# om-ai-lab/OmChat

Measured on AMD Instinct MI355X. Metric: images/sec prefill + decode tokens/sec, OmChat-13B TP=1/8; p50 TTFT, higher is better.
Workload: dtype bf16

## Files before the change

omchat_amd/csrc/capi.hip:

```cpp
#include "kernels.h"
#include <stdlib.h>
#include "../../include/omchat_hip.h"
#include <math.h>
#include <vector>

#define S(x) ((hipStream_t)(x))
#if OMCHAT_EXPERIMENTS
int g_launch_any_order = 0;
#endif

extern "C" int omchat_op_gemm(int dtype, const void* A, int lda, const void* W, int ldw, void* C, int ldc, int M, int N, int K,
                              const void* bias, const void* ls, const void* resid, int ldr, int epi, int force_tile, void* stream) {
  GemmArgs g{A, lda, W, ldw, C, ldc, M, N, K, bias, ls, resid, ldr, epi, force_tile, nullptr, 0, -1};
  return launch_gemm(dtype, g, S(stream));
}

extern "C" int omchat_op_gemm_fused(int dtype, const void* A, int lda, const void* W, int ldw, void* C, int ldc, int M, int N, int K,
                                    const void* bias, const void* ls, const void* resid, int ldr, int epi, int force_tile, const float* row_scale,
                                    const float* rs_stats, int rs_ld, int rs_nslots, int rs_dim, float rs_eps,
                                    float* stats, int stats_ld, int* nslots, void* stream) {
  GemmArgs g{A, lda, W, ldw, C, ldc, M, N, K, bias, ls, resid, ldr, epi, force_tile, nullptr, 0, -1};
  g.row_scale = row_scale; g.stats = stats; g.stats_ld = stats_ld; g.stats_nslots = nslots;
  g.rs_stats = rs_stats; g.rs_ld = rs_ld; g.rs_nslots = rs_nslots; g.rs_dim = rs_dim; g.rs_eps = rs_eps;
  return launch_gemm(dtype, g, S(stream));
}
extern "C" int omchat_op_stats_finish(const float* stats, int ld, int slot0, int nslots, int ngroups, int rows, int dim, float eps, float* out, void* stream) {
  return launch_stats_finish(stats, ld, slot0, nslots, ngroups, rows, dim, eps, out, S(stream));
}
extern "C" int omchat_op_row_sumsq(int dtype, const void* x, int ldx, int rows, int H, float* stats, void* stream) {
  return launch_row_sumsq(dtype, x, ldx, rows, H, stats, S(stream));
}
extern "C" int omchat_op_fold_cols(int dtype, const void* W, const void* n, void* out, int rows, int cols, void* stream) {
  return launch_fold_cols(dtype, W, n, out, rows, cols, S(stream));
}
extern "C" int omchat_op_vit_knorm_slots(int dtype, void* k, int ld, const void* wk, int rows, int C, int C_total, float eps, const float* stats, int stats_ld,
                                         int nslots, float* sumsq_q, void* stream) {
  return launch_vit_knorm_slots(dtype, k, ld, wk, rows, C, C_total, eps, stats, stats_ld, nslots, sumsq_q, S(stream));
}
extern "C" int omchat_op_mha_qnorm(int dtype, const void* qkv, int B, int Sq, int H, const float* sumsq, int stride, int dim, const void* wq,
                                   float eps, float q_scale, void* out, void* stream) {
  OM_CHECK(qkv && out && sumsq && wq, "null argument");
  AttnArgs a{};
  const int64_t row = (int64_t)3 * H * 128;
  a.Q = qkv; a.q_sb = Sq * row; a.q_sh = 128; a.q_sr = row;
  a.K = (const char*)qkv + (size_t)H * 128 * 2; a.k_sb = a.q_sb; a.k_sh = 128; a.k_sr = row;
  a.V = (const char*)qkv + (size_t)2 * H * 128 * 2; a.v_sb = a.q_sb; a.v_sh = 128; a.v_sr = row;
  a.O = out; a.o_sb = (int64_t)Sq * H * 128; a.o_sh = 128; a.o_sr = (int64_t)H * 128;
  a.batch = B; a.q_heads = H; a.kv_heads = H; a.Sq = Sq; a.Skv = Sq; a.kv_len = nullptr; a.causal = 0; a.q_pos0 = 0;
  a.scale = 1.0f;
  a.qn_sumsq = sumsq; a.qn_stride = stride; a.qn_dim = dim; a.qn_w = wq; a.qn_eps = eps; a.qn_scale = q_scale;
  return launch_attn_prefill(dtype, a, S(stream));
}

extern "C" int omchat_op_set_tuning(int key, int value) {
  const char* allow = getenv("OMCHAT_ALLOW_TUNING");
  if (!allow || allow[0] != '1') {
    omchat_set_error("omchat_op_set_tuning: process-global test / measurement hook; set OMCHAT_ALLOW_TUNING=1 to use it (see include/omchat_hip.h)");
    return 1;
  }
  if (key == 0) { gemm_set_skew(value); return 0; }
  if (key == 1) { gemv_set_force_mfma(value); return 0; }
  if (key == 5) { gemm_set_autotune(value); return 0; }
  if (key == 4) { model_set_ar_min_rows(value); return 0; }
  if (key == 6) { model_set_pack_replica(value); return 0; }
  if (key == 8) { attn_set_v2(value); return 0; }
  if (key == 9) { model_set_fuse_peer_norm(value); return 0; }
  if (key == 10) { attn_set_tpw(value); return 0; }
  if (key == 11) { gemv_set_no_xs(value); return 0; }
  if (key == 12) { attn_set_klds(value); return 0; }
  if (key == 25) { attn_set_dma(value); return 0; }
  if (key == 26) { attn_set_dma_slots(value); return 0; }
  if (key == 27) { attn_set_dma_rot(value); return 0; }
  if (key == 28) { gemv_set_skew(value); return 0; }
  if (key == 29) { model_set_tp_f32(value); return 0; }
  if (key == 30) { attn_set_hsplit(value); return 0; }
  if (key == 33) { attn_set_mha_xcd(value); return 0; }
  if (key == 16) { gemv_set_norm_loop(value); return 0; }
  if (key == 17) { gemv_set_rows_balance(value); return 0; }
  if (key == 19) { attn_set_merge_mid_min(value); return 0; }
  if (key == 21) { attn_set_merge_dg(value); return 0; }
  if (key == 13) { gemm_set_persist(value); return 0; }
  if (key == 14) { model_set_norm_in_gemv(value); return 0; }
  if (key == 22) { model_set_fuse_attn_oproj(value); return 0; }
  if (key == 23) { model_set_decode_layer(value); return 0; }
  if (key == 24) { gemv_set_dyn(value); return 0; }
  if (key == 34) { gemv_set_shard_shapes(value); return 0; }
  if (key == 35) { model_set_shard_as_tp1(value); return 0; }
  if (key == 36) { attn_set_kg(value); return 0; }
  if (key == 37) { gemm_set_wide_store(value); return 0; }
  if (key == 43) { gemm_set_skip_dead(value); return 0; }
  if (key == 44) { model_set_vit_fused(value); return 0; }
  if (key == 45) { model_set_tp_sp(value); return 0; }
  if (key == 46) { attn_set_peel(value); return 0; }
  if (key == 47) { attn_set_kv8_tpw(value); return 0; }
  if (key == 48) { attn_set_kv8_fuse(value); return 0; }
  if (key == 49) { model_set_extend_attn(value); return 0; }
  if (key == 38) { gemv_set_gu_rr(value); return 0; }
  if (key == 39) { gemv_set_longk_direct(value); return 0; }
  if (key == 40) { norm_set_wave(value); return 0; }
#if OMCHAT_EXPERIMENTS
  if (key == 41) { g_launch_any_order = value; return 0; }
  if (key == 42) { model_set_ao_oproj(value); return 0; }
#endif
  omchat_set_error("omchat_op_set_tuning: unknown key");
  return 1;
}

extern "C" int omchat_allreduce_noop(void*, void*, size_t, int, void*) { return 0; }

extern "C" int omchat_gemm_tune_load(const char* path) { OM_CHECK(path, "null path"); return gemm_tune_load(path); }
extern "C" int omchat_gemm_tune_dump(const char* path) { OM_CHECK(path, "null path"); return gemm_tune_dump(path); }
extern "C" long omchat_gemm_tune_runs(void) { return gemm_tune_runs(); }

extern "C" size_t omchat_op_gemm_sk_ws(void) { return gemm_sk_ws_bytes(); }

extern "C" int omchat_op_gemm_sk(int dtype, const void* A, int lda, const void* W, int ldw, void* C, int ldc, int M, int N, int K,
                                 const void* bias, const void* ls, const void* resid, int ldr, int epi, int force_tile, void* ws,
                                 size_t ws_bytes, int stream_k, void* stream) {
  GemmArgs g{A, lda, W, ldw, C, ldc, M, N, K, bias, ls, resid, ldr, epi, force_tile, ws, ws_bytes, stream_k};
  return launch_gemm(dtype, g, S(stream));
}

extern "C" int omchat_op_gemv(int dtype, const void* X, int ldx, const void* W, int ldw, void* Y, int ldy, int b, int N, int K,
                              const void* bias, const void* resid, int ldr, int epi, int out_f32, void* stream) {
  GemvArgs g{X, ldx, W, ldw, Y, ldy, b, N, K, bias, resid, ldr, epi, out_f32};
  return launch_gemv(dtype, g, S(stream));
}

extern "C" int omchat_op_gemv_norm(int dtype, const void* X, const void* W, int ldw, void* Y, int N, int K, const void* norm_w, float eps,
                                   const void* bias, int epi, int out_f32, void* stream) {
  OM_CHECK(X && W && Y && norm_w, "null argument");
  GemvArgs g{X, K, W, ldw, Y, N, 1, N, K, bias, nullptr, 0, epi, out_f32};
  g.norm_w = norm_w; g.norm_eps = eps;
  return launch_gemv(dtype, g, S(stream));
}

extern "C" int omchat_op_gemv_packed(int dtype, const void* X, int ldx, const void* W, int ldw, void* Y, int ldy, int b, int N, int K,
                                     const void* bias, int epi, int out_f32, int ksplit, int w_packed, int y_packed, void* stream) {
  OM_CHECK(b >= 1 && b <= 32 && K % 64 == 0, "1 <= b <= 32, K % 64 == 0");
  const int NB = b > 16 ? 2 : 1;
  void *xp = nullptr, *wp = nullptr;
  OM_HIP(hipMalloc(&xp, (size_t)NB * 16 * K * 2));
  int rc = launch_pack_x(dtype, X, ldx, b, K, xp, S(stream));
  if (rc == 0 && w_packed) {
    if (hipMalloc(&wp, (size_t)N * K * 2) != hipSuccess) { hipFree(xp); omchat_set_error("hipMalloc failed"); return 2; }
    rc = launch_pack_w(dtype, W, ldw, N, K, wp, S(stream));
  }
  if (rc == 0) {
    GemvArgs g{xp, K, w_packed ? wp : W, ldw, Y, ldy, b, N, K, bias, nullptr, 0, epi, out_f32, ksplit, 0, nullptr, 1, w_packed, y_packed};
    rc = launch_gemv(dtype, g, S(stream));
  }
  hipStreamSynchronize(S(stream));
  hipFree(xp); if (wp) hipFree(wp);
  return rc;
}
extern "C" int omchat_op_pack_x(int dtype, const void* X, int ldx, int b, int K, void* out, void* stream) { return launch_pack_x(dtype, X, ldx, b, K, out, S(stream)); }

extern "C" int omchat_op_gemm_fp8(int dtype, const void* A8, const float* a_scale, const void* W8, const float* w_scale, void* C, int ldc, int M,
                                  int N, int K, const void* bias, const void* resid, int ldr, int epi, void* stream) {
  GemmArgs g{A8, K, W8, K, C, ldc, M, N, K, bias, nullptr, resid, ldr, epi, 0, nullptr, 0, -1, 1, a_scale, w_scale};
  return launch_gemm(dtype, g, S(stream));
}
extern "C" int omchat_op_quant_rows_fp8(int dtype, const void* x, const void* norm_w, float eps, void* y8, float* scale, int rows, int H, void* stream) {
  if (norm_w) return launch_rmsnorm_q8(dtype, x, H, norm_w, y8, H, scale, rows, H, eps, S(stream));
  return launch_quant_rows_q8(dtype, x, H, y8, H, scale, rows, H, S(stream));
}

extern "C" int omchat_op_resid_rmsnorm(int dtype, void* x, int ldx, const float* part, int ks, const void* w, void* xn, int ldn, int rows, int H,
                                       float eps, int pack_nb, void* stream) {
  OM_CHECK(x && part, "null argument");
  return launch_resid_rmsnorm(dtype, x, ldx, part, ks, w, xn, ldn, rows, H, eps, S(stream), pack_nb);
}
extern "C" int omchat_op_rmsnorm(int dtype, const void* x, const void* w, void* y, int rows, int H, float eps, void* stream) {
// ... 339 lines not shown
```

omchat_amd/csrc/gemm.hip:

```cpp
#include "kernels.h"
#include <array>
#include <stdio.h>
#include <stdlib.h>
#include <limits.h>
#include <algorithm>
#include <map>
#include <mutex>

namespace {

int g_gemm_wide_store = 1;
int g_gemm_skip_dead = 1;

struct GemmP {
  const void* A; const void* W; void* C; const void* bias; const void* ls; const void* resid;
  int lda, ldw, ldc, ldr, M, N, K;
  const float* a_scale; const float* w_scale;
  int wide_store;
  int skip_dead;
  const float* row_scale;
  float* stats; int stats_ld;
  const float* rs_stats; int rs_ld, rs_nslots; float rs_inv_dim, rs_eps;
  int rs_dma;
};

constexpr int GROUP_M = 4;
__device__ __forceinline__ int xcd_remap(int bid, int nwg) {
  const int xcd = bid & 7, q8 = nwg >> 3, r8 = nwg & 7;
  return (xcd < r8 ? xcd * (q8 + 1) : r8 * (q8 + 1) + (xcd - r8) * q8) + (bid >> 3);
}
__device__ __forceinline__ void tile_coords_id(int wgid, int M, int N, int BM, int BN, int& m0, int& n0) {
  const int tiles_m = (M + BM - 1) / BM, tiles_n = (N + BN - 1) / BN;
  const int per_group = GROUP_M * tiles_n;
  const int g = wgid / per_group, in_g = wgid % per_group;
  const int rows_here = tiles_m - g * GROUP_M < GROUP_M ? tiles_m - g * GROUP_M : GROUP_M;
  m0 = (g * GROUP_M + in_g % rows_here) * BM;
  n0 = (in_g / rows_here) * BN;
}
__device__ __forceinline__ void tile_coords(int M, int N, int BM, int BN, int& m0, int& n0) {
  tile_coords_id(xcd_remap(blockIdx.x, gridDim.x), M, N, BM, BN, m0, n0);
}

typedef const __attribute__((address_space(1))) void* gptr_t;
typedef __attribute__((address_space(3))) void* lptr_t;

template <typename T> __device__ __forceinline__ unsigned short bits16(T v) { return __builtin_bit_cast(unsigned short, v); }
template <typename T> __device__ __forceinline__ float from_bits16(unsigned short v) { return tof(__builtin_bit_cast(T, v)); }
template <typename T> __device__ __forceinline__ u32x2 pack4(float a, float b, float c, float d) {
  typename V8<T>::half_type h = {fromf<T>(a), fromf<T>(b), fromf<T>(c), fromf<T>(d)};
  return __builtin_bit_cast(u32x2, h);
}
template <typename T> __device__ __forceinline__ f32x4 unpack4(u32x2 w) {
  const typename V8<T>::half_type h = __builtin_bit_cast(typename V8<T>::half_type, w);
  return (f32x4){tof(h[0]), tof(h[1]), tof(h[2]), tof(h[3])};
}
template <typename T> __device__ __forceinline__ f32x4 load4(const T* p) {
  return unpack4<T>(*reinterpret_cast<const u32x2*>(p));
}

template <typename T, int MR, int NR, int EPI_, bool F8 = false>
__device__ __forceinline__ void gemm_epilogue(const GemmP& p, f32x4 (&acc)[MR][NR], int rowu_, int colu_, int fg, int fr, const float* rs_lds = nullptr) {
#pragma clang fp contract(off)
  constexpr bool STATS = EPI_ == EPI_LS_RESID_STATS || EPI_ == EPI_NONE_STATS;
  constexpr int EPI = EPI_ == EPI_LS_RESID_STATS ? EPI_LS_RESID : (EPI_ == EPI_NONE_STATS ? EPI_NONE : EPI_);
  const int rowu = __builtin_amdgcn_readfirstlane(rowu_), colu = __builtin_amdgcn_readfirstlane(colu_);
  const int rows_valid = p.M - rowu < MR * 16 ? p.M - rowu : MR * 16;
  if (rows_valid <= 0) return;
  if (p.row_scale || rs_lds) {
    float rs[MR];
#pragma unroll
    for (int i = 0; i < MR; ++i) {
      const int row = rowu + i * 16 + fr;
      rs[i] = rs_lds ? rs_lds[i * 16 + fr] : p.row_scale[row < p.M ? row : p.M - 1];
    }
#pragma unroll
    for (int i = 0; i < MR; ++i)
#pragma unroll
      for (int j = 0; j < NR; ++j) acc[i][j] *= rs[i];
  }
  float ssq[MR];
#pragma unroll
  for (int i = 0; i < MR; ++i) ssq[i] = 0.f;
  if constexpr (F8) {
    float sa[MR];
#pragma unroll
    for (int i = 0; i < MR; ++i) { const int row = rowu + i * 16 + fr; sa[i] = p.a_scale[row < p.M ? row : p.M - 1]; }
#pragma unroll
    for (int j = 0; j < NR; ++j) {
      const int col = colu + j * 16 + 4 * fg;
      const f32x4 sw = col < p.N ? *reinterpret_cast<const f32x4*>(p.w_scale + col) : (f32x4){0.f, 0.f, 0.f, 0.f};
#pragma unroll
      for (int i = 0; i < MR; ++i) acc[i][j] *= sw * sa[i];
    }
  }
// ... 91 lines not shown
#pragma unroll
          for (int jj = 0; jj < JG; jj += 2) {
            const int j = j0 + jj;
            if (j + 1 < NR && colu + j * 16 < p.N) {
              const bool mine = colu + (j + (fg & 1)) * 16 + 4 * (fg & ~1) < p.N;
              const int cw = (fr * p.ldc + 4 * (fg & ~1)) * 2 + (colu + (j + (fg & 1)) * 16) * 2;
              const u32x2 a = out4(i, jj), b = out4(i, jj + 1);
              const auto s0 = __builtin_amdgcn_permlane16_swap(a[0], b[0], false, false);
              const auto s1 = __builtin_amdgcn_permlane16_swap(a[1], b[1], false, false);
              const u32x4 w = {s0[0], s1[0], s0[1], s1[1]};
              if (mine) __builtin_amdgcn_raw_buffer_store_b128(w, crs, cw + i * 16 * p.ldc * 2, 0, 0);
            }
          }
        }
      } else {
#pragma unroll
      for (int jj = 0; jj < JG; ++jj) {
        const int j = j0 + jj;
        const int col = colu + j * 16 + 4 * fg;
        if (j < NR && col < p.N) {
          const int cj = c_lane + (colu + j * 16) * 2;
#pragma unroll
          for (int i = 0; i < MR; ++i) __builtin_amdgcn_raw_buffer_store_b64(out4(i, jj), crs, cj + i * 16 * p.ldc * 2, 0, 0);
        }
      }
      }
    }
    if constexpr (STATS) {
      if (colu < p.N) {
        const int slot = colu / (NR * 16);
#pragma unroll
        for (int i = 0; i < MR; ++i) {
          float v = ssq[i];
          v += __shfl_xor(v, 16);
          v += __shfl_xor(v, 32);
          const int row = rowu + i * 16 + fr;
          if (fg == 0 && row < p.M) p.stats[(size_t)slot * p.stats_ld + row] = v;
        }
      }
    }
  }
}

template <int BM, int NT>
__device__ __forceinline__ void tile_row_scale_prefetch(const GemmP& p, int m0, float* Ls) {
  const int lane = threadIdx.x & 63, wave = __builtin_amdgcn_readfirstlane((int)threadIdx.x >> 6);
  constexpr int G = (BM + 63) / 64;
  for (int pc = wave; pc < p.rs_nslots * G; pc += NT / 64) {
    const int sl = pc / G, g = pc - sl * G;
    int r = g * 64 + lane; r = r < BM ? r : BM - 1;
    int row = m0 + r; row = row < p.M ? row : p.M - 1;
    __builtin_amdgcn_global_load_lds((gptr_t)(p.rs_stats + (size_t)sl * p.rs_ld + row), (lptr_t)(Ls + sl * (G * 64) + g * 64), 4, 0, 0);
  }
}

template <int BM, int NT>
__device__ __forceinline__ void tile_row_scale(const GemmP& p, int m0, float* L, const float* Ls) {
  constexpr int TPR = NT >= 2 * BM ? 2 : 1;
  constexpr int G64 = (BM + 63) / 64 * 64;
  const int tid = threadIdx.x, h = tid / BM, r = tid % BM;
  if (h < TPR) {
    int row = m0 + r; row = row < p.M ? row : p.M - 1;
    const int per = (p.rs_nslots + TPR - 1) / TPR, s0 = h * per, s1 = s0 + per < p.rs_nslots ? s0 + per : p.rs_nslots;
    const float* base = p.rs_stats + row;
    float t = 0.f;
    for (int c0 = s0; c0 < s1; c0 += 16) {
      float v[16];
#pragma unroll
      for (int k = 0; k < 16; ++k) v[k] = c0 + k < s1 ? (Ls ? Ls[(c0 + k) * G64 + r] : base[(size_t)(c0 + k) * p.rs_ld]) : 0.f;
#pragma unroll
      for (int k = 0; k < 16; ++k) t += v[k];
    }
    L[h * BM + r] = t;
  }
  __syncthreads();
  if (tid < BM) {
    float t = L[tid];
    if (TPR == 2) t += L[BM + tid];
    L[tid] = rsqrtf(t * p.rs_inv_dim + p.rs_eps);
  }
  __syncthreads();
}

template <typename T, int BM, int BN, int WM, int WN, int EPI>
__global__ __launch_bounds__(WM* WN * 64) void gemm_kernel(GemmP p) {
  constexpr int NT = WM * WN * 64;
  constexpr int WTM = BM / WM, WTN = BN / WN;
  constexpr int MR = WTM / 16, NR = WTN / 16;
  constexpr int A_BYTES = BM * 128, B_BYTES = BN * 128, STAGE = A_BYTES + B_BYTES;
  constexpr int A_ROUNDS = (BM * 8 + NT - 1) / NT, B_ROUNDS = (BN * 8 + NT - 1) / NT;
  static_assert((BM * 8) % 64 == 0 && (BN * 8) % 64 == 0 && WTM % 16 == 0 && WTN % 16 == 0, "tile geometry");
  typedef typename V8<T>::type frag_t;
  extern __shared__ __attribute__((aligned(256))) char smem[];

  const int tid = threadIdx.x;
  const int lane = tid & 63;
  const int wave = __builtin_amdgcn_readfirstlane(tid >> 6);
  const int wm = wave / WN, wn = wave % WN;

  int m0, n0;
  tile_coords(p.M, p.N, BM, BN, m0, n0);

  const T* __restrict__ A = (const T*)p.A;
  const T* __restrict__ W = (const T*)p.W;

  const T* a_src[A_ROUNDS];
  const T* b_src[B_ROUNDS];
#pragma unroll
  for (int i = 0; i < A_ROUNDS; ++i) {
    const int lin = i * NT + tid, row = lin >> 3, pc = lin & 7;
    const int c = pc ^ ((row >> 1) & 7);
    int gr = m0 + row; gr = gr < p.M ? gr : p.M - 1;
    a_src[i] = A + (size_t)gr * p.lda + c * 8;
  }
#pragma unroll
  for (int i = 0; i < B_ROUNDS; ++i) {
    const int lin = i * NT + tid, row = lin >> 3, pc = lin & 7;
    const int c = pc ^ ((row >> 1) & 7);
    int gr = n0 + row; gr = gr < p.N ? gr : p.N - 1;
    b_src[i] = W + (size_t)gr * p.ldw + c * 8;
  }

  auto stage = [&](int buf, int kt) {
    char* base = smem + buf * STAGE;
#pragma unroll
    for (int i = 0; i < A_ROUNDS; ++i)
      if ((i + 1) * NT <= BM * 8 || i * NT + wave * 64 < BM * 8)
        __builtin_amdgcn_global_load_lds((gptr_t)(a_src[i] + kt * 64), (lptr_t)(base + (i * NT + wave * 64) * 16), 16, 0, 0);
#pragma unroll
    for (int i = 0; i < B_ROUNDS; ++i)
      if ((i + 1) * NT <= BN * 8 || i * NT + wave * 64 < BN * 8)
        __builtin_amdgcn_global_load_lds((gptr_t)(b_src[i] + kt * 64), (lptr_t)(base + A_BYTES + (i * NT + wave * 64) * 16), 16, 0, 0);
  };

  const int fr = lane & 15, fg = lane >> 4;
  const int swz = (fr >> 1) & 7;
  int a_off[2], b_off[2];
#pragma unroll
  for (int s = 0; s < 2; ++s) {
    const int pc = ((s * 4 + fg) ^ swz) * 16;
    a_off[s] = (wm * WTM + fr) * 128 + pc;
    b_off[s] = A_BYTES + (wn * WTN + fr) * 128 + pc;
  }

  f32x4 acc[MR][NR];
#pragma unroll
  for (int i = 0; i < MR; ++i)
#pragma unroll
    for (int j = 0; j < NR; ++j) acc[i][j] = (f32x4){0.f, 0.f, 0.f, 0.f};

  const int nk = p.K / 64;
  float* const rs_ls = reinterpret_cast<float*>(smem + 2 * STAGE);
  if (p.rs_stats && p.rs_dma) tile_row_scale_prefetch<BM, NT>(p, m0, rs_ls);
  const bool wave_live = !p.skip_dead || m0 + wm * WTM < p.M;
  stage(0, 0);
  for (int t = 0; t < nk; ++t) {
    asm volatile("s_waitcnt vmcnt(0)" ::: "memory");
    __syncthreads();
    if (t + 1 < nk) stage((t + 1) & 1, t + 1);
    if (!wave_live) continue;
    const char* base = smem + (t & 1) * STAGE;
#pragma unroll
    for (int s = 0; s < 2; ++s) {
      frag_t af[MR], bf[NR];
#pragma unroll
      for (int i = 0; i < MR; ++i) af[i] = *reinterpret_cast<const frag_t*>(base + a_off[s] + i * 16 * 128);
#pragma unroll
      for (int j = 0; j < NR; ++j) bf[j] = *reinterpret_cast<const frag_t*>(base + b_off[s] + j * 16 * 128);
#pragma unroll
      for (int i = 0; i < MR; ++i)
#pragma unroll
        for (int j = 0; j < NR; ++j) acc[i][j] = mfma16(bf[j], af[i], acc[i][j]);
    }
  }

  const float* rs_lds = nullptr;
  if (p.rs_stats) {
    __syncthreads();
    tile_row_scale<BM, NT>(p, m0, reinterpret_cast<float*>(smem), p.rs_dma ? rs_ls : nullptr);
    rs_lds = reinterpret_cast<const float*>(smem) + wm * WTM;
  }
  gemm_epilogue<T, MR, NR, EPI>(p, acc, m0 + wm * WTM, n0 + wn * WTN, fg, fr, rs_lds);
}


#ifndef OMCHAT_F8_SCALED
#define OMCHAT_F8_SCALED 1
#endif
template <typename T>
__device__ __forceinline__ f32x4 mma_frag_f8x128(typename V8<T>::type a0, typename V8<T>::type a1, typename V8<T>::type b0, typename V8<T>::type b1, f32x4 c) {
  typedef int i32x4 __attribute__((ext_vector_type(4)));
  typedef int i32x8 __attribute__((ext_vector_type(8)));
  const i32x4 al = __builtin_bit_cast(i32x4, a0), ah = __builtin_bit_cast(i32x4, a1), bl = __builtin_bit_cast(i32x4, b0), bh = __builtin_bit_cast(i32x4, b1);
  const i32x8 a = {al[0], al[1], al[2], al[3], ah[0], ah[1], ah[2], ah[3]};
  const i32x8 b = {bl[0], bl[1], bl[2], bl[3], bh[0], bh[1], bh[2], bh[3]};
  return __builtin_amdgcn_mfma_scale_f32_16x16x128_f8f6f4(a, b, c, 0 , 0 , 0, 0x7F7F7F7F, 0, 0x7F7F7F7F);
}

template <typename T, bool F8>
__device__ __forceinline__ f32x4 mma_frag(typename V8<T>::type a, typename V8<T>::type b, f32x4 c) {
  if constexpr (F8) {
    typedef long l2 __attribute__((ext_vector_type(2)));
    const l2 a2 = __builtin_bit_cast(l2, a), b2 = __builtin_bit_cast(l2, b);
    c = __builtin_amdgcn_mfma_f32_16x16x32_fp8_fp8(a2[0], b2[0], c, 0, 0, 0);
    return __builtin_amdgcn_mfma_f32_16x16x32_fp8_fp8(a2[1], b2[1], c, 0, 0, 0);
  } else {
    return mfma16(a, b, c);
  }
}

template <typename T, bool F8 = false>
__device__ __forceinline__ void gemm8_segment(const GemmP& p, int m0, int n0, int kt0, int kt1, char* smem, f32x4 (&acc)[8][4],
                                              bool prologue_issued = false, bool has_next = false, int next_m0 = 0, int next_n0 = 0) {
  constexpr int SLOT = 128 * 128;
  constexpr int STAGE = 4 * SLOT;
  constexpr int ES = F8 ? 1 : 2;
  typedef typename V8<T>::type frag_t;

  const int tid = threadIdx.x, lane = tid & 63;
  const int wave = __builtin_amdgcn_readfirstlane(tid >> 6);
  const int wm = wave >> 2, wn = wave & 3;

  const char* __restrict__ A = (const char*)p.A;
  const char* __restrict__ W = (const char*)p.W;

  const char* a_src[2][2];
  const char* b_src[2][2];
  auto set_src = [&](int tm0, int tn0) {
#pragma unroll
    for (int i = 0; i < 2; ++i) {
      const int lin = i * 512 + tid, rho = lin >> 3, pc = lin & 7;
      const int c = pc ^ ((rho >> 1) & 7);
#pragma unroll
      for (int h = 0; h < 2; ++h) {
        int gr = tm0 + (rho >> 6) * 128 + h * 64 + (rho & 63); gr = gr < p.M ? gr : p.M - 1;
        a_src[h][i] = A + (size_t)gr * p.lda * ES + c * 16;
        int gc = tn0 + (rho >> 5) * 64 + h * 32 + (rho & 31); gc = gc < p.N ? gc : p.N - 1;
// ... 212 lines not shown
          covered = e < tile_end ? e : tile_end;
        }
      }
      gemm_epilogue<T, 8, 4, EPI>(p, acc, m0 + wm * 128, n0 + wn * 64, fg, fr);
    }
    it += k1 - k0;
  }
}

int g_gemm_persist = 0;
int g_gemm_skew = 0;
constexpr size_t SK_SLAB_BYTES = 65536 * 4;
constexpr int SK_MAX_WG = 256;

template <typename T, int EPI>
int launch_cfg8(const GemmArgs& a, hipStream_t stream) {
  constexpr int LDS = 2 * 4 * 128 * 128;
  auto kern = gemm8_kernel<T, EPI>;
  auto kern_p = gemm8p_kernel<T, EPI>;
  auto kern_sk = gemm8_sk_kernel<T, EPI>;
  static PerDeviceOnce attr_set;
  const int n_cu = device_cus();
  if (attr_set.first()) {
    OM_HIP(hipFuncSetAttribute((const void*)kern, hipFuncAttributeMaxDynamicSharedMemorySize, 160 * 1024));
    OM_HIP(hipFuncSetAttribute((const void*)kern_p, hipFuncAttributeMaxDynamicSharedMemorySize, LDS));
    OM_HIP(hipFuncSetAttribute((const void*)kern_sk, hipFuncAttributeMaxDynamicSharedMemorySize, LDS));
  }
  GemmP p{a.A, a.W, a.C, a.bias, a.ls, a.resid, a.lda, a.ldw, a.ldc, a.ldr, a.M, a.N, a.K, nullptr, nullptr, g_gemm_wide_store, g_gemm_skip_dead, a.row_scale, a.stats, a.stats_ld, a.rs_stats, a.rs_ld, a.rs_nslots, a.rs_dim > 0 ? 1.0f / (float)a.rs_dim : 0.f, a.rs_eps, 0};
  const int tiles = cdiv(a.M, 256) * cdiv(a.N, 256);
  if (a.stats_nslots) *a.stats_nslots = cdiv(a.N, 64);
  const int rs_bytes = a.rs_stats ? a.rs_nslots * 256 * 4 : 0;
  p.rs_dma = rs_bytes > 0 && LDS + rs_bytes <= 160 * 1024;
  const int lds_main = p.rs_dma ? LDS + rs_bytes : LDS;
  const int KT = a.K / 64;
  const int G = n_cu < SK_MAX_WG ? n_cu : SK_MAX_WG;
  int R = tiles % G;
  const bool have_ws = a.sk_ws && a.sk_ws_bytes >= (size_t)G * SK_SLAB_BYTES + 4096;
  const bool use_sk = a.stream_k > 0 && have_ws && !a.rs_stats && R > 0 && R * 10 < G * 9 && (long)R * KT >= 4L * G && KT >= 8;
  if (a.stream_k > 0 && !use_sk && !have_ws) { omchat_set_error("launch_gemm: stream-K requested without workspace"); return 1; }
  if (!use_sk) R = 0;
  const int n_dp = tiles - R;
  if (n_dp > G && g_gemm_persist && R == 0 && G >= 8 && !a.rs_stats) hipLaunchKernelGGL(kern_p, dim3(G & ~7), dim3(512), LDS, stream, p, n_dp);
  else if (n_dp > 0) hipLaunchKernelGGL(kern, dim3(n_dp), dim3(512), lds_main, stream, p, g_gemm_skew);
  if (R > 0) {
    unsigned* flags = reinterpret_cast<unsigned*>((char*)a.sk_ws + (size_t)G * SK_SLAB_BYTES);
    OM_HIP(hipMemsetAsync(flags, 0, 4096, stream));
    SkP sk{n_dp, R, (float*)a.sk_ws, flags, flags + 1000};
    hipLaunchKernelGGL(kern_sk, dim3(G), dim3(512), LDS, stream, p, sk);
  }
  OM_LAUNCH_CHECK();
  return 0;
}

template <typename T, int EPI>
int launch_cfg8_f8(const GemmArgs& a, hipStream_t stream) {
  constexpr int LDS = 2 * 4 * 128 * 128;
  auto kern = gemm8_kernel<T, EPI, true>;
  auto kern_p = gemm8p_kernel<T, EPI, true>;
  static PerDeviceOnce attr_set;
  const int n_cu = device_cus();
  if (attr_set.first()) {
    OM_HIP(hipFuncSetAttribute((const void*)kern, hipFuncAttributeMaxDynamicSharedMemorySize, LDS));
    OM_HIP(hipFuncSetAttribute((const void*)kern_p, hipFuncAttributeMaxDynamicSharedMemorySize, LDS));
  }
  GemmP p{a.A, a.W, a.C, a.bias, a.ls, a.resid, a.lda, a.ldw, a.ldc, a.ldr, a.M, a.N, a.K, a.a_scale, a.w_scale, g_gemm_wide_store, g_gemm_skip_dead, a.row_scale, a.stats, a.stats_ld, a.rs_stats, a.rs_ld, a.rs_nslots, a.rs_dim > 0 ? 1.0f / (float)a.rs_dim : 0.f, a.rs_eps, 0};
  const int tiles = cdiv(a.M, 256) * cdiv(a.N, 256);
  if (tiles > n_cu && g_gemm_persist && n_cu >= 8 && !a.rs_stats) hipLaunchKernelGGL(kern_p, dim3(n_cu & ~7), dim3(512), LDS, stream, p, tiles);
  else hipLaunchKernelGGL(kern, dim3(tiles), dim3(512), LDS, stream, p, 0);
  OM_LAUNCH_CHECK();
  return 0;
}

template <typename T, int BM, int BN, int WM, int WN, int EPI>
int launch_cfg(const GemmArgs& a, hipStream_t stream) {
  constexpr int LDS = 2 * (BM + BN) * 128;
  auto kern = gemm_kernel<T, BM, BN, WM, WN, EPI>;
  static PerDeviceOnce attr_set;
  constexpr int LDS_MAX = LDS + 32 * 1024 <= 160 * 1024 ? LDS + 32 * 1024 : 160 * 1024;
  if (attr_set.first()) OM_HIP(hipFuncSetAttribute((const void*)kern, hipFuncAttributeMaxDynamicSharedMemorySize, LDS_MAX));
  GemmP p{a.A, a.W, a.C, a.bias, a.ls, a.resid, a.lda, a.ldw, a.ldc, a.ldr, a.M, a.N, a.K, nullptr, nullptr, g_gemm_wide_store, g_gemm_skip_dead, a.row_scale, a.stats, a.stats_ld, a.rs_stats, a.rs_ld, a.rs_nslots, a.rs_dim > 0 ? 1.0f / (float)a.rs_dim : 0.f, a.rs_eps, 0};
  const int grid = cdiv(a.M, BM) * cdiv(a.N, BN);
  if (a.stats_nslots) *a.stats_nslots = cdiv(a.N, BN / WN);
  const int rs_bytes = a.rs_stats ? a.rs_nslots * ((BM + 63) / 64 * 64) * 4 : 0;
  p.rs_dma = rs_bytes > 0 && LDS + rs_bytes <= LDS_MAX;
  hipLaunchKernelGGL(kern, dim3(grid), dim3(WM * WN * 64), p.rs_dma ? LDS + rs_bytes : LDS, stream, p);
  OM_LAUNCH_CHECK();
  return 0;
}

struct TileCfg { int id, bm, bn, slots; float eff; };
static const TileCfg kTiles[] = {{2, 256, 256, 256, 1.00f}, {3, 256, 192, 256, 0.90f}, {1, 128, 128, 512, 0.60f}};

static int pick_tile(int M, int N, int epi) {
  if ((long)cdiv(M, 256) * cdiv(N, 256) >= 3 * 256) return 2;
  int best = 2;
  float best_cost = 1e30f;
  for (const TileCfg& t : kTiles) {
    if (epi == EPI_SWIGLU && (t.bn / 4) % 32 != 0) continue;
    const long tiles = (long)cdiv(M, t.bm) * cdiv(N, t.bn);
    const long rounds = (tiles + t.slots - 1) / t.slots;
    const float cost = (float)rounds * (float)(t.bm * t.bn) / t.eff * (t.slots == 512 ? 2.0f : 1.0f) + 0.02f * 65536.f * (float)rounds;
    if (cost < best_cost) { best_cost = cost; best = t.id; }
  }
  return best;
}

template <typename T, int EPI>
int launch_epi(const GemmArgs& a, hipStream_t stream) {
  const int tile = a.force_tile ? a.force_tile : pick_tile(a.M, a.N, EPI);
  switch (tile) {
    case 1: return launch_cfg<T, 128, 128, 2, 2, EPI>(a, stream);
    case 3: return launch_cfg<T, 256, 192, 2, 4, EPI>(a, stream);
    case 4: return launch_cfg<T, 224, 256, 2, 4, EPI>(a, stream);
    case 5: return launch_cfg<T, 192, 256, 2, 4, EPI>(a, stream);
    case 6: return launch_cfg<T, 256, 256, 2, 4, EPI>(a, stream);
    case 7: return launch_cfg<T, 256, 192, 4, 3, EPI>(a, stream);
    case 8: return launch_cfg<T, 256, 256, 4, 4, EPI>(a, stream);
    case 9: return launch_cfg<T, 192, 256, 3, 4, EPI>(a, stream);
    case 10: if constexpr (EPI != EPI_SWIGLU) return launch_cfg<T, 192, 224, 4, 2, EPI>(a, stream); else break;
    case 11: if constexpr (EPI != EPI_SWIGLU) return launch_cfg<T, 192, 224, 6, 2, EPI>(a, stream); else break;
    case 12: case 13:
      if constexpr (EPI != EPI_SWIGLU) {
        const int G = device_cus(), rt = cdiv(a.M, 256), ct = cdiv(a.N, 256);
        const int full = (rt * ct) / G;
        const int ct_main = full >= 1 ? std::min(ct, (full * G) / rt) : 0;
        const int n_main = ct_main * 256, n_tail = a.N - n_main;
        if (n_main > 0 && n_tail > 0 && (long)cdiv(a.M, 192) * cdiv(n_tail, 224) <= G) {
          GemmArgs m = a, t = a;
          m.N = n_main; m.force_tile = 2;
          const size_t es = 2;
          t.N = n_tail; t.force_tile = a.force_tile == 12 ? 10 : 11;
          t.W = (const char*)a.W + (size_t)n_main * a.ldw * es;
          t.C = (char*)a.C + (size_t)n_main * es;
          if (a.bias) t.bias = (const char*)a.bias + (size_t)n_main * es;
          if (a.ls) t.ls = (const char*)a.ls + (size_t)n_main * es;
          if (a.resid) t.resid = (const char*)a.resid + (size_t)n_main * es;
          int ns_main = 0, ns_tail = 0;
          if (a.stats) { t.stats = a.stats + (size_t)(n_main / 64) * a.stats_ld; m.stats_nslots = &ns_main; t.stats_nslots = &ns_tail; }
          int rc = launch_cfg8<T, EPI>(m, stream);
          if (rc) return rc;
          rc = t.force_tile == 10 ? launch_cfg<T, 192, 224, 4, 2, EPI>(t, stream) : launch_cfg<T, 192, 224, 6, 2, EPI>(t, stream);
          if (a.stats_nslots) *a.stats_nslots = ns_main + ns_tail;
          return rc;
        }
      }
      break;
    default: return launch_cfg8<T, EPI>(a, stream);
  }
  return launch_cfg8<T, EPI>(a, stream);
}

template <typename T>
int launch_t(const GemmArgs& a, hipStream_t stream) {
  switch (a.epi) {
    case EPI_LS_RESID_STATS: return launch_epi<T, EPI_LS_RESID_STATS>(a, stream);
    case EPI_NONE_STATS: {
      GemmArgs b = a;
      if (b.force_tile != 2 && b.force_tile != 6 && b.force_tile != 8 && b.force_tile != 9 && b.force_tile != 7) b.force_tile = 2;
      return launch_epi<T, EPI_NONE_STATS>(b, stream);
    }
    case EPI_NONE: return launch_epi<T, EPI_NONE>(a, stream);
    case EPI_GELU: return launch_epi<T, EPI_GELU>(a, stream);
    case EPI_LS_RESID: return launch_epi<T, EPI_LS_RESID>(a, stream);
    case EPI_RESID: return launch_epi<T, EPI_RESID>(a, stream);
    case EPI_SWIGLU: return launch_epi<T, EPI_SWIGLU>(a, stream);
    case EPI_F32OUT: return a.force_tile == 1 ? launch_cfg<T, 128, 128, 2, 2, EPI_F32OUT>(a, stream) : launch_cfg8<T, EPI_F32OUT>(a, stream);
  }
  omchat_set_error("launch_gemm: bad epilogue");
  return 1;
}

}

void gemm_set_skew(int v) { g_gemm_skew = v; }
void gemm_set_persist(int v) { g_gemm_persist = v; }
void gemm_set_wide_store(int v) { g_gemm_wide_store = v; }
void gemm_set_skip_dead(int v) { g_gemm_skip_dead = v; }

static int g_autotune = getenv("OMCHAT_GEMM_AUTOTUNE") ? atoi(getenv("OMCHAT_GEMM_AUTOTUNE")) : 1;
void gemm_set_autotune(int v) { g_autotune = v; }

static std::mutex g_tune_mu;
static std::map<std::array<int, 5>, int> g_tuned;
static long g_tune_runs = 0;

int gemm_tune_load(const char* path) {
  FILE* f = fopen(path, "r");
  if (!f) return -1;
  std::lock_guard<std::mutex> lock(g_tune_mu);
  int n = 0, a, b, c, d, e, t;
  char line[256];
  while (fgets(line, sizeof line, f)) {
    if (line[0] == '#') continue;
    if (sscanf(line, "%d %d %d %d %d %d", &a, &b, &c, &d, &e, &t) == 6 && t >= 1 && t <= 13) { g_tuned[{a, b, c, d, e}] = t; ++n; }
  }
  fclose(f);
  return n;
}
int gemm_tune_dump(const char* path) {
  FILE* f = fopen(path, "w");
  if (!f) return -1;
  std::lock_guard<std::mutex> lock(g_tune_mu);
  fprintf(f, "# omchat_amd GEMM tile choices measured on this device: dtype*8+epi ceil(M/256) N K ldc tile\n");
  for (auto& kv : g_tuned) fprintf(f, "%d %d %d %d %d %d\n", kv.first[0], kv.first[1], kv.first[2], kv.first[3], kv.first[4], kv.second);
  fclose(f);
  return (int)g_tuned.size();
}
long gemm_tune_runs() { return g_tune_runs; }

static std::map<std::array<int, 5>, int> g_guess;

static int tuned_tile(int dtype, const GemmArgs& a, hipStream_t stream) {
  if (a.epi == EPI_LS_RESID_STATS || a.epi == EPI_NONE_STATS) {
    GemmArgs b = a;
    b.epi = a.epi == EPI_NONE_STATS ? EPI_NONE : EPI_LS_RESID;
    b.stats = nullptr;
    return tuned_tile(dtype, b, stream);
  }
  const std::array<int, 5> key{dtype * 8 + a.epi, cdiv(a.M, 256), a.N, a.K, a.ldc};
  std::lock_guard<std::mutex> lock(g_tune_mu);
  auto it = g_tuned.find(key);
  if (it != g_tuned.end()) return it->second;
  it = g_guess.find(key);
  if (it != g_guess.end()) return it->second;
  const int heuristic = pick_tile(a.M, a.N, a.epi);
  if ((double)a.M * a.N * a.K < 4e9) return g_guess[key] = heuristic;
  {
    int best_d = INT_MAX, best_t = 0;
    for (auto& kv : g_tuned) {
      const auto& k = kv.first;
      if (k[0] != key[0] || k[2] != key[2] || k[3] != key[3] || k[4] != key[4]) continue;
      const int d = k[1] > key[1] ? k[1] - key[1] : key[1] - k[1];
      if (d < best_d) { best_d = d; best_t = kv.second; }
    }
    if (best_t && best_d <= std::max(1, key[1] / 8)) return g_guess[key] = best_t;
  }
  hipStreamCaptureStatus cs = hipStreamCaptureStatusNone;
  if (hipStreamIsCapturing(stream, &cs) != hipSuccess || cs != hipStreamCaptureStatusNone) return heuristic;
  GemmArgs t = a;
  t.M = a.M < 8192 ? a.M : 8192;
  void* scratch = nullptr;
  if (hipMalloc(&scratch, (size_t)t.M * a.ldc * 2) != hipSuccess) { (void)hipGetLastError(); return g_guess[key] = heuristic; }
  t.C = scratch;
  constexpr size_t FLUSH_BYTES = (size_t)384 << 20;
  void* flush = nullptr;
  if (hipMalloc(&flush, FLUSH_BYTES) != hipSuccess) { (void)hipGetLastError(); flush = nullptr; }
  hipEvent_t e0, e1;
  (void)hipEventCreate(&e0); (void)hipEventCreate(&e1);
  ++g_tune_runs;
  int cands[9] = {2, 8, 9, 7, 3, 10, 11, 12, 13};
  int best = heuristic;
  float best_ms = 1e30f;
  for (int c : cands) {
    if ((c == 3 || c >= 10) && a.epi == EPI_SWIGLU) continue;
    t.force_tile = c;
    bool ok = true;
    auto run = [&]() {
      int rc = 1;
      if (dtype == OMCHAT_F16) rc = launch_t<f16>(t, stream);
      else if (dtype == OMCHAT_BF16) rc = launch_t<bf16>(t, stream);
      ok = ok && rc == 0;
    };
    run();
    float ms = 1e30f;
    for (int i = 0; i < 3 && ok; ++i) {
      if (flush) (void)hipMemsetAsync(flush, i, FLUSH_BYTES, stream);
      (void)hipEventRecord(e0, stream);
      run();
      (void)hipEventRecord(e1, stream);
      if (hipEventSynchronize(e1) != hipSuccess) { (void)hipGetLastError(); ok = false; break; }
      float one = 0.f;
      (void)hipEventElapsedTime(&one, e0, e1);
      ms = one < ms ? one : ms;
    }
    if (!ok) continue;
    if (getenv("OMCHAT_TUNE_LOG")) fprintf(stderr, "[omchat tune] M=%d N=%d K=%d epi=%d tile %d: %.1f us\n", a.M, a.N, a.K, a.epi, c, ms * 1e3f);
    if (ms < best_ms) { best_ms = ms; best = c; }
  }
  (void)hipEventDestroy(e0); (void)hipEventDestroy(e1);
  (void)hipFree(scratch);
  if (flush) (void)hipFree(flush);
  return g_tuned[key] = best;
}
size_t gemm_sk_ws_bytes() { return (size_t)SK_MAX_WG * SK_SLAB_BYTES + 4096; }

template <typename T>
static int launch_f8_t(const GemmArgs& a, hipStream_t stream) {
  switch (a.epi) {
    case EPI_NONE: return launch_cfg8_f8<T, EPI_NONE>(a, stream);
    case EPI_GELU: return launch_cfg8_f8<T, EPI_GELU>(a, stream);
    case EPI_LS_RESID: return launch_cfg8_f8<T, EPI_LS_RESID>(a, stream);
    case EPI_RESID: return launch_cfg8_f8<T, EPI_RESID>(a, stream);
    case EPI_SWIGLU: return launch_cfg8_f8<T, EPI_SWIGLU>(a, stream);
  }
  omchat_set_error("launch_gemm: bad epilogue");
  return 1;
}

int launch_gemm(int dtype, const GemmArgs& a, hipStream_t stream) {
  OM_CHECK(a.M > 0 && a.N > 0 && a.K > 0, "empty problem");
  if (a.f8) {
    OM_CHECK(a.K % 128 == 0 && a.lda % 16 == 0 && a.ldw % 16 == 0 && a.a_scale && a.w_scale, "fp8 GEMM: K % 128, lda / ldw % 16 bytes, both scale vectors");
    OM_CHECK(((uintptr_t)a.A & 15) == 0 && ((uintptr_t)a.W & 15) == 0 && a.ldc % 4 == 0 && ((uintptr_t)a.C & 7) == 0 &&
             (!a.resid || (a.ldr % 4 == 0 && ((uintptr_t)a.resid & 7) == 0)), "fp8 GEMM: A / W 16-byte, C / residual 8-byte aligned with row strides % 4");
    OM_CHECK(a.epi != EPI_SWIGLU || a.N % 32 == 0, "SwiGLU epilogue needs N % 32 == 0");
    OM_CHECK(a.N % 4 == 0 && ((uintptr_t)a.bias & 7) == 0 && ((uintptr_t)a.ls & 7) == 0 && ((uintptr_t)a.w_scale & 15) == 0,
             "fp8 GEMM: N % 4, bias / layer-scale 8-byte and w_scale 16-byte aligned");
    if (dtype == OMCHAT_F16) return launch_f8_t<f16>(a, stream);
    if (dtype == OMCHAT_BF16) return launch_f8_t<bf16>(a, stream);
    omchat_set_error("launch_gemm: bad dtype");
    return 1;
  }
  OM_CHECK(a.K % 64 == 0, "K must be a multiple of 64");
  OM_CHECK(a.lda % 8 == 0 && a.ldw % 8 == 0, "lda/ldw must be multiples of 8 elements (16-byte rows)");
  OM_CHECK(a.ldc % 4 == 0 && (!a.resid || a.ldr % 4 == 0) && ((uintptr_t)a.C & 7) == 0 && ((uintptr_t)a.resid & 7) == 0,
           "C / residual: 8-byte aligned base, row stride a multiple of 4 elements (8-byte epilogue accesses)");
  OM_CHECK(((uintptr_t)a.A & 15) == 0 && ((uintptr_t)a.W & 15) == 0, "A/W must be 16-byte aligned");
  OM_CHECK(a.epi != EPI_SWIGLU || a.N % 32 == 0, "SwiGLU epilogue needs N % 32 == 0");
  OM_CHECK((a.epi != EPI_LS_RESID && a.epi != EPI_LS_RESID_STATS) || a.ls, "layer-scale epilogue needs ls");
  OM_CHECK((a.epi != EPI_LS_RESID_STATS && a.epi != EPI_NONE_STATS) || (a.stats && a.stats_ld >= a.M), "statistics epilogue: stats [slots][stats_ld] (slot-major), stats_ld >= M");
  OM_CHECK(!a.rs_stats || (a.rs_nslots >= 1 && a.rs_ld >= a.M && a.rs_dim > 0 && !a.row_scale), "row statistics: slot-major [rs_nslots][rs_ld >= M], rs_dim > 0, not together with row_scale");
  OM_CHECK(a.N % 4 == 0 && ((uintptr_t)a.bias & 7) == 0 && ((uintptr_t)a.ls & 7) == 0,
           "N must be a multiple of 4 and bias / layer-scale 8-byte aligned (the epilogue owns four consecutive columns per lane)");
  OM_CHECK(dtype == OMCHAT_F16 || dtype == OMCHAT_BF16, "bad dtype");
  GemmArgs b = a;
  if (a.epi == EPI_F32OUT) {
    OM_CHECK(a.ldc % 4 == 0 && ((uintptr_t)a.C & 15) == 0 && !a.bias && !a.resid, "fp32-output GEMM: C 16-byte aligned, ldc % 4 == 0, no bias / residual");
    b.force_tile = (long)cdiv(a.M, 256) * cdiv(a.N, 256) < 64 ? 1 : 2;
    b.stream_k = -1;
  } else
  if (!a.force_tile && g_autotune && a.stream_k <= 0) b.force_tile = tuned_tile(dtype, a, stream);
  if (dtype == OMCHAT_F16) return launch_t<f16>(b, stream);
  return launch_t<bf16>(b, stream);
}
```

omchat_amd/csrc/kernels.h:

```cpp
#pragma once
#ifndef OMCHAT_EXPERIMENTS
#define OMCHAT_EXPERIMENTS 0
#endif
#include "common.h"
#if OMCHAT_EXPERIMENTS
#include <hip/hip_ext.h>
extern int g_launch_any_order;
#undef hipLaunchKernelGGL
#define hipLaunchKernelGGL(kernelName, numBlocks, numThreads, memPerBlock, streamId, ...)                                                      \
  do {                                                                                                                                         \
    if (g_launch_any_order)                                                                                                                    \
      hipExtLaunchKernelGGL((kernelName), dim3(numBlocks), dim3(numThreads), (memPerBlock), (streamId), nullptr, nullptr, hipExtAnyOrderLaunch, \
                            __VA_ARGS__);                                                                                                      \
    else                                                                                                                                       \
      hipLaunchKernelGGLInternal((kernelName), numBlocks, numThreads, memPerBlock, streamId, __VA_ARGS__);                                     \
  } while (0)
#endif

enum {
  EPI_NONE = 0,
  EPI_GELU = 1,
  EPI_LS_RESID = 2,
  EPI_RESID = 3,
  EPI_SWIGLU = 4,
  EPI_PARTIAL = 5,
  EPI_F32OUT = 6,
  EPI_LS_RESID_STATS = 7,
  EPI_NONE_STATS = 8,
};
struct GemmArgs {
  const void* A; int lda;
  const void* W; int ldw;
  void* C; int ldc;
  int M, N, K;
  const void* bias;
  const void* ls;
  const void* resid;
  int ldr;
  int epi;
  int force_tile;
  void* sk_ws; size_t sk_ws_bytes;
  int stream_k;
  int f8;
  const float* a_scale; const float* w_scale;
  const float* row_scale = nullptr;
  const float* rs_stats = nullptr; int rs_ld = 0, rs_nslots = 0, rs_dim = 0; float rs_eps = 0.f;
  float* stats = nullptr; int stats_ld = 0; int* stats_nslots = nullptr;
};
int launch_gemm(int dtype, const GemmArgs& a, hipStream_t stream);
int launch_stats_finish(const float* stats, int ld, int slot0, int nslots, int ngroups, int rows, int dim, float eps, float* out, hipStream_t s);
int launch_row_sumsq(int dtype, const void* x, int ldx, int rows, int H, float* stats, hipStream_t s);
size_t gemm_sk_ws_bytes();
void gemm_set_skew(int v);
void gemm_set_persist(int v);
void gemm_set_wide_store(int v);
void gemm_set_skip_dead(int v);

struct GemvArgs {
  const void* X; int ldx;
  const void* W; int ldw;
  void* Y; int ldy;
  int b, N, K;
  const void* bias;
  const void* resid; int ldr;
  int epi;
  int out_f32;
  int ksplit;
  int force_mfma;
  const float* w_scale;
  int x_packed;
  int w_packed;
  int y_packed;
  const void* norm_w; float norm_eps;
  void* dyn_ctr = nullptr;
  void* y_pack = nullptr;
  unsigned long long* dbg = nullptr;
};
int launch_pack_x(int dtype, const void* X, int ldx, int b, int K, void* out, hipStream_t s);
int launch_pack_w(int dtype, const void* W, int ldw, int N, int K, void* out, hipStream_t s);
int launch_gemv(int dtype, const GemvArgs& a, hipStream_t stream);
int launch_gemv_wait(int dtype, const GemvArgs& a, const unsigned* flags, unsigned epoch, int nflags, unsigned* err, int mode, hipStream_t s);
int launch_quant_fp8_rows(int dtype, const void* W, int ldw, int N, int K, void* W8, int ld8, float* scale, hipStream_t stream);
void gemv_set_force_mfma(int v);
int gemv_get_force_mfma();
void gemm_set_autotune(int v);
int gemm_tune_load(const char* path);
int gemm_tune_dump(const char* path);
long gemm_tune_runs();
void model_set_ar_min_rows(int v);
void model_set_tp_f32(int v);
void model_set_pack_replica(int v);
void model_set_norm_in_gemv(int v);
void model_set_vit_fused(int v);
void model_set_tp_sp(int v);
int launch_fold_cols(int dtype, const void* W, const void* n, void* out, int rows, int cols, hipStream_t s);

int launch_layernorm(int dtype, const void* x, int ldx, const void* w, const void* b, void* y, int ldy, int rows, int H, float eps, hipStream_t stream);
int launch_rmsnorm(int dtype, const void* x, int ldx, const void* w, void* y, int ldy, int rows, int H, float eps, hipStream_t s, int pack_nb = 0);
int launch_rmsnorm_q8(int dtype, const void* x, int ldx, const void* w, void* y8, int ldy, float* scale, int rows, int H, float eps, hipStream_t s);
int launch_quant_rows_q8(int dtype, const void* x, int ldx, void* y8, int ldy, float* scale, int rows, int H, hipStream_t s);
int launch_resid_rmsnorm(int dtype, void* x, int ldx, const float* part, int ks, const void* w, void* xn, int ldn, int rows, int H, float eps,
                         hipStream_t s, int pack_nb = 0);
int launch_resid16_norm(int dtype, void* x, int ldx, const void* y, int ldy, const void* w, const void* b, void* xn, int ldn, int rows, int H, float eps,
                        hipStream_t s);
int launch_vit_qknorm(int dtype, void* qkv, int ld, const void* wq, const void* wk, int rows, int C, int C_total,
                      float eps, float q_scale, const float* sumsq_in, hipStream_t s, int only_k = 0);
int launch_vit_qk_sumsq(int dtype, const void* qkv, int ld, int rows, int C, float* sumsq_out, hipStream_t s);
int launch_vit_knorm_slots(int dtype, void* k, int ld, const void* wk, int rows, int C, int C_total, float eps, const float* stats, int stats_ld, int nslots,
                           float* sumsq_q, hipStream_t s);
struct AttnArgs {
  const void* Q; int64_t q_sb, q_sh, q_sr;
  const void* K; int64_t k_sb, k_sh, k_sr;
  const void* V; int64_t v_sb, v_sh, v_sr;
  void* O; int64_t o_sb, o_sh, o_sr;
  int batch, q_heads, kv_heads;
  int Sq, Skv;
  const int* kv_len;
  const int* kv_start;
  int causal;
  int q_pos0;
  float scale;
  int head_dim;
  const float* qn_sumsq = nullptr; int qn_stride = 0, qn_dim = 0; const void* qn_w = nullptr; float qn_eps = 0.f, qn_scale = 1.f;
};
int launch_attn_prefill(int dtype, const AttnArgs& a, hipStream_t s);
int launch_attn_uniform_rows(int dtype, const AttnArgs& a, hipStream_t s);
void attn_set_v2(int v);
void model_set_fuse_peer_norm(int v);
void attn_set_tpw(int v);
void attn_set_klds(int v);
void attn_set_dma(int v);
void attn_set_dma_slots(int v);
void attn_set_dma_rot(int v);
void attn_set_hsplit(int v);
void attn_set_mha_xcd(int v);
void attn_set_kg(int v);
void attn_set_peel(int v);
void attn_set_kv8_tpw(int v);
void attn_set_kv8_fuse(int v);
// ... 169 lines not shown
```

Measured before the change: 342.7.

## Add software-pipelined 320x256 GEMM tile with interleaved MFMA/LDS/DMA scheduling

Adds a new 320x256 GEMM tile config (tile 14) for NONE/GELU/SWIGLU epilogues. It uses a restructured main loop: LDS fragment reads for the next k-step are register-prefetched during the current MFMAs, global-to-LDS DMA for step t+2 is overlapped, and sched_group_barrier hints interleave the instructions. The row-scale statistics prefetch moves into a spare region of the freed stage buffer, so LDS does not grow. The tile joins the autotune candidate list and can be disabled with a tuning key. This adds code complexity and a larger register footprint.

```diff
diff --git a/omchat_amd/csrc/capi.hip b/omchat_amd/csrc/capi.hip
--- a/omchat_amd/csrc/capi.hip
+++ b/omchat_amd/csrc/capi.hip
@@ -89,6 +89,7 @@
   if (key == 36) { attn_set_kg(value); return 0; }
   if (key == 37) { gemm_set_wide_store(value); return 0; }
   if (key == 43) { gemm_set_skip_dead(value); return 0; }
+  if (key == 50) { gemm_set_tile320(value); return 0; }
   if (key == 44) { model_set_vit_fused(value); return 0; }
   if (key == 45) { model_set_tp_sp(value); return 0; }
   if (key == 46) { attn_set_peel(value); return 0; }
diff --git a/omchat_amd/csrc/gemm.hip b/omchat_amd/csrc/gemm.hip
--- a/omchat_amd/csrc/gemm.hip
+++ b/omchat_amd/csrc/gemm.hip
@@ -6,10 +6,13 @@
 #include <algorithm>
 #include <map>
 #include <mutex>
+#include <type_traits>
+#include <utility>
 
 namespace {
 
 int g_gemm_wide_store = 1;
+int g_gemm_tile320 = 1;
 int g_gemm_skip_dead = 1;
 
 struct GemmP {
@@ -267,8 +270,43 @@
   __syncthreads();
 }
 
+template <int... I, typename F>
+__device__ __forceinline__ void static_for_impl(std::integer_sequence<int, I...>, F&& f) { (f(std::integral_constant<int, I>{}), ...); }
+template <int N, typename F>
+__device__ __forceinline__ void static_for(F&& f) { static_for_impl(std::make_integer_sequence<int, N>{}, f); }
+
+template <int BM, int NT>
+__device__ __forceinline__ void tile_row_scale_loop(const GemmP& p, int m0, float* L, const float* Ls) {
+  constexpr int G64 = (BM + 63) / 64 * 64;
+  const int tid = threadIdx.x;
+  const int per = (p.rs_nslots + 1) / 2;
+  for (int w = tid; w < 2 * BM; w += NT) {
+    const int h = w / BM, r = w % BM;
+    int row = m0 + r; row = row < p.M ? row : p.M - 1;
+    const int s0 = h * per, s1 = s0 + per < p.rs_nslots ? s0 + per : p.rs_nslots;
+    const float* base = p.rs_stats + row;
+    float t = 0.f;
+    for (int c0 = s0; c0 < s1; c0 += 16) {
+      float v[16];
+#pragma unroll
+      for (int k = 0; k < 16; ++k) v[k] = c0 + k < s1 ? (Ls ? Ls[(c0 + k) * G64 + r] : base[(size_t)(c0 + k) * p.rs_ld]) : 0.f;
+#pragma unroll
+      for (int k = 0; k < 16; ++k) t += v[k];
+    }
+    L[h * BM + r] = t;
+  }
+  __syncthreads();
+  for (int r = tid; r < BM; r += NT) {
+    float t = L[r];
+    t += L[BM + r];
+    L[r] = rsqrtf(t * p.rs_inv_dim + p.rs_eps);
+  }
+  __syncthreads();
+}
+
 template <typename T, int BM, int BN, int WM, int WN, int EPI>
 __global__ __launch_bounds__(WM* WN * 64) void gemm_kernel(GemmP p) {
+  constexpr bool PIPE = BM == 320;
   constexpr int NT = WM * WN * 64;
   constexpr int WTM = BM / WM, WTN = BN / WN;
   constexpr int MR = WTM / 16, NR = WTN / 16;
@@ -335,9 +373,100 @@
     for (int j = 0; j < NR; ++j) acc[i][j] = (f32x4){0.f, 0.f, 0.f, 0.f};
 
   const int nk = p.K / 64;
+  const bool wave_live = !p.skip_dead || m0 + wm * WTM < p.M;
+  if constexpr (PIPE) {
+    static_assert((BM * 8) % NT == 0 && (BN * 8) % NT == 0, "whole staging rounds: every wave issues A_ROUNDS + B_ROUNDS loads per stage");
+    constexpr int LPS = A_ROUNDS + B_ROUNDS;
+    float* const rs_ls = reinterpret_cast<float*>(smem + (nk & 1) * STAGE + 4096);
+    const int t_stats = nk >= 2 ? nk - 2 : 0;
+    const char* const Ab = (const char*)p.A;
+    const char* const Wb = (const char*)p.W;
+    unsigned a_of[A_ROUNDS];
+#pragma unroll
+    for (int i = 0; i < A_ROUNDS; ++i) {
+      const int lin = i * NT + tid, row = lin >> 3, c = (lin & 7) ^ ((row >> 1) & 7);
+      int gr = m0 + row; gr = gr < p.M ? gr : p.M - 1;
+      a_of[i] = ((unsigned)gr * (unsigned)p.lda + c * 8) * 2u;
+    }
+    const unsigned b_of = ((unsigned)(n0 + (tid >> 3)) * (unsigned)p.ldw + ((tid & 7) ^ ((tid >> 4) & 7)) * 8) * 2u;
+    static_assert((NT / 8) % 16 == 0, "the swizzle term (row >> 1) & 7 is the same in every staging round");
+    auto stage32 = [&](int buf, int kt) {
+      char* base = smem + buf * STAGE;
+      const char* ak = Ab + (size_t)kt * 128;
+      const char* wk = Wb + (size_t)kt * 128;
+#pragma unroll
+      for (int i = 0; i < A_ROUNDS; ++i) __builtin_amdgcn_global_load_lds((gptr_t)(ak + a_of[i]), (lptr_t)(base + (i * NT + wave * 64) * 16), 16, 0, 0);
+#pragma unroll
+      for (int i = 0; i < B_ROUNDS; ++i)
+        __builtin_amdgcn_global_load_lds((gptr_t)(wk + (size_t)i * (NT / 8) * p.ldw * 2 + b_of), (lptr_t)(base + A_BYTES + (i * NT + wave * 64) * 16), 16, 0, 0);
+    };
+    frag_t a[MR], b[NR];
+    auto ld = [&](const char* q) { return *reinterpret_cast<const frag_t*>(q); };
+    auto half = [&](const char* nb, int ns, bool rd_next, auto ndma_c) {
+      constexpr int NDMA = decltype(ndma_c)::value;
+      static_for<MR>([&](auto ic) {
+        constexpr int i = decltype(ic)::value;
+#pragma unroll
+        for (int j = 0; j < NR; ++j) acc[i][j] = mfma16(b[j], a[i], acc[i][j]);
+        if (rd_next) a[i] = ld(nb + (a_off[0] ^ (ns << 6)) + i * 16 * 128);
+        constexpr int nd = NDMA * (i + 1) / MR - NDMA * i / MR;
+        if constexpr (nd > 0) __builtin_amdgcn_sched_group_barrier(0x010, nd, 0);
+        __builtin_amdgcn_sched_group_barrier(0x008, NR, 0);
+        __builtin_amdgcn_sched_group_barrier(0x100, 1, 0);
+      });
+      if (rd_next) {
+#pragma unroll
+        for (int j = 0; j < NR; ++j) b[j] = ld(nb + (b_off[0] ^ (ns << 6)) + j * 16 * 128);
+      }
+    };
+    stage32(0, 0);
+    if (nk > 1) {
+      stage32(1, 1);
+      asm volatile("s_waitcnt vmcnt(%0)" ::"n"(LPS) : "memory");
+    } else {
+      asm volatile("s_waitcnt vmcnt(0)" ::: "memory");
+    }
+    __syncthreads();
+    auto step = [&](int t, auto live_c, auto full_c) {
+      constexpr bool LIVE = decltype(live_c)::value, FULL = decltype(full_c)::value;
+      const char* base = smem + (t & 1) * STAGE;
+      const char* nbase = smem + ((t + 1) & 1) * STAGE;
+      if constexpr (LIVE) half(base, 1, true, std::integral_constant<int, 0>{});
+      __builtin_amdgcn_sched_barrier(0);
+      asm volatile("s_waitcnt lgkmcnt(0)" ::: "memory");
+      asm volatile("s_waitcnt vmcnt(0)" ::: "memory");
+      __builtin_amdgcn_s_barrier();
+      __builtin_amdgcn_sched_barrier(0);
+      if (FULL || t + 2 < nk) stage32(t & 1, t + 2);
+      if (!FULL && t == t_stats && p.rs_stats && p.rs_dma) tile_row_scale_prefetch<BM, NT>(p, m0, rs_ls);
+      if constexpr (LIVE) half(nbase, 0, FULL || t + 1 < nk, std::integral_constant<int, FULL ? LPS : 0>{});
+      __builtin_amdgcn_sched_barrier(0);
+    };
+    auto loop = [&](auto live_c) {
+      if constexpr (decltype(live_c)::value) {
+#pragma unroll
+        for (int i = 0; i < MR; ++i) a[i] = ld(smem + a_off[0] + i * 16 * 128);
+#pragma unroll
+        for (int j = 0; j < NR; ++j) b[j] = ld(smem + b_off[0] + j * 16 * 128);
+      }
+      int t = 0;
+      for (; t + 2 < nk; ++t) step(t, live_c, std::true_type{});
+      for (; t < nk; ++t) step(t, live_c, std::false_type{});
+    };
+    if (wave_live) loop(std::true_type{});
+    else loop(std::false_type{});
+    const float* rs_lds = nullptr;
+    if (p.rs_stats) {
+      asm volatile("s_waitcnt vmcnt(0)" ::: "memory");
+      __syncthreads();
+      tile_row_scale_loop<BM, NT>(p, m0, reinterpret_cast<float*>(smem), p.rs_dma ? rs_ls : nullptr);
+      rs_lds = reinterpret_cast<const float*>(smem) + wm * WTM;
+    }
+    gemm_epilogue<T, MR, NR, EPI>(p, acc, m0 + wm * WTM, n0 + wn * WTN, fg, fr, rs_lds);
+    return;
+  }
   float* const rs_ls = reinterpret_cast<float*>(smem + 2 * STAGE);
   if (p.rs_stats && p.rs_dma) tile_row_scale_prefetch<BM, NT>(p, m0, rs_ls);
-  const bool wave_live = !p.skip_dead || m0 + wm * WTM < p.M;
   stage(0, 0);
   for (int t = 0; t < nk; ++t) {
     asm volatile("s_waitcnt vmcnt(0)" ::: "memory");
@@ -716,6 +845,12 @@
   const int grid = cdiv(a.M, BM) * cdiv(a.N, BN);
   if (a.stats_nslots) *a.stats_nslots = cdiv(a.N, BN / WN);
   const int rs_bytes = a.rs_stats ? a.rs_nslots * ((BM + 63) / 64 * 64) * 4 : 0;
+  if constexpr (BM == 320) {
+    p.rs_dma = rs_bytes > 0 && 4096 + rs_bytes <= LDS / 2;
+    hipLaunchKernelGGL(kern, dim3(grid), dim3(WM * WN * 64), LDS, stream, p);
+    OM_LAUNCH_CHECK();
+    return 0;
+  }
   p.rs_dma = rs_bytes > 0 && LDS + rs_bytes <= LDS_MAX;
   hipLaunchKernelGGL(kern, dim3(grid), dim3(WM * WN * 64), p.rs_dma ? LDS + rs_bytes : LDS, stream, p);
   OM_LAUNCH_CHECK();
@@ -779,6 +914,11 @@
         }
       }
       break;
+    case 14:
+      if constexpr (EPI == EPI_NONE || EPI == EPI_GELU || EPI == EPI_SWIGLU) {
+        if (a.N % 256 == 0) return launch_cfg<T, 320, 256, 2, 4, EPI>(a, stream);
+      }
+      break;
     default: return launch_cfg8<T, EPI>(a, stream);
   }
   return launch_cfg8<T, EPI>(a, stream);
@@ -810,6 +950,7 @@
 void gemm_set_persist(int v) { g_gemm_persist = v; }
 void gemm_set_wide_store(int v) { g_gemm_wide_store = v; }
 void gemm_set_skip_dead(int v) { g_gemm_skip_dead = v; }
+void gemm_set_tile320(int v) { g_gemm_tile320 = v; }
 
 static int g_autotune = getenv("OMCHAT_GEMM_AUTOTUNE") ? atoi(getenv("OMCHAT_GEMM_AUTOTUNE")) : 1;
 void gemm_set_autotune(int v) { g_autotune = v; }
@@ -826,7 +967,7 @@
   char line[256];
   while (fgets(line, sizeof line, f)) {
     if (line[0] == '#') continue;
-    if (sscanf(line, "%d %d %d %d %d %d", &a, &b, &c, &d, &e, &t) == 6 && t >= 1 && t <= 13) { g_tuned[{a, b, c, d, e}] = t; ++n; }
+    if (sscanf(line, "%d %d %d %d %d %d", &a, &b, &c, &d, &e, &t) == 6 && t >= 1 && t <= 14) { g_tuned[{a, b, c, d, e}] = t; ++n; }
   }
   fclose(f);
   return n;
@@ -882,11 +1023,12 @@
   hipEvent_t e0, e1;
   (void)hipEventCreate(&e0); (void)hipEventCreate(&e1);
   ++g_tune_runs;
-  int cands[9] = {2, 8, 9, 7, 3, 10, 11, 12, 13};
+  int cands[10] = {2, 8, 9, 7, 3, 10, 11, 12, 13, 14};
   int best = heuristic;
   float best_ms = 1e30f;
   for (int c : cands) {
-    if ((c == 3 || c >= 10) && a.epi == EPI_SWIGLU) continue;
+    if ((c == 3 || (c >= 10 && c <= 13)) && a.epi == EPI_SWIGLU) continue;
+    if (c == 14 && ((a.epi != EPI_NONE && a.epi != EPI_GELU && a.epi != EPI_SWIGLU) || a.N % 256)) continue;
     t.force_tile = c;
     bool ok = true;
     auto run = [&]() {
@@ -963,7 +1105,10 @@
     b.force_tile = (long)cdiv(a.M, 256) * cdiv(a.N, 256) < 64 ? 1 : 2;
     b.stream_k = -1;
   } else
-  if (!a.force_tile && g_autotune && a.stream_k <= 0) b.force_tile = tuned_tile(dtype, a, stream);
+  if (!a.force_tile && g_autotune && a.stream_k <= 0) {
+    b.force_tile = tuned_tile(dtype, a, stream);
+    if (b.force_tile >= 14 && !g_gemm_tile320) b.force_tile = 2;
+  }
   if (dtype == OMCHAT_F16) return launch_t<f16>(b, stream);
   return launch_t<bf16>(b, stream);
 }
diff --git a/omchat_amd/csrc/kernels.h b/omchat_amd/csrc/kernels.h
--- a/omchat_amd/csrc/kernels.h
+++ b/omchat_amd/csrc/kernels.h
@@ -55,6 +55,7 @@
 void gemm_set_persist(int v);
 void gemm_set_wide_store(int v);
 void gemm_set_skip_dead(int v);
+void gemm_set_tile320(int v);
 
 struct GemvArgs {
   const void* X; int ldx;
```

Result: no change. 344.6 (median of 6 runs) (+0.5%).
